# vocdoni/gnark-crypto-primitives

Hardware: AMD Instinct MI355X
Metric: proofs/sec, Arbo-160 Poseidon SMT-verifier circuit, Groth16/BN254 (higher is better)
Workload: dtype u32x8 Montgomery (254-bit integer)

## Files before the change

gnark_crypto_primitives_amd/csrc/solve.hip:

```cpp
#include <cstdlib>

#include "zkmi_internal.h"
#include "emul.h"
#include "ff29.h"
#include "ff29_asm.h"
#include "modinv30.h"

namespace zk {

__device__ __forceinline__ Fr fmul(const Fr& a, const Fr& b) {
  Fr r;
  pack_canonical<Fr29Params>(r.v,
                             mul_asm(unpack29<Fr29Params>(a.v), unpack29<Fr29Params>(b.v)));
  return r;
}
__device__ __forceinline__ Fr f_one() {
  Fr r;
#pragma unroll
  for (int i = 0; i < 8; i++) r.v[i] = Fr29Params::k261(i);
  return r;
}
__device__ Fr finv(const Fr& a) {
  Fr t, c;
  modinv30<ModInvFr>(t.v, a.v);
// ... 20 lines not shown
__device__ __forceinline__ uint32_t limb_at(const Fr& v, uint32_t pos, uint32_t wd) {
  if (pos >= 256) return 0;
  const uint32_t lo = v.v[pos >> 5], hi = (pos >> 5) < 7 ? v.v[(pos >> 5) + 1] : 0u;
  const uint64_t two = ((uint64_t)hi << 32) | lo;
  return (uint32_t)(two >> (pos & 31)) & ((1u << wd) - 1u);
}


template <int BANK, bool WAIT, bool NT>
__device__ __forceinline__ void st_acc(Fr* base, size_t row, size_t b, size_t Bp, const Fr& x) {
  uint4* p0 = reinterpret_cast<uint4*>(base) + row * 2 * Bp + b;
  uint4* p1 = p0 + Bp;
#define ZK_ST_ACC_ASM(A0, A1, A2, A3, A4, A5, A6, A7, LO, HI, NT_)                                 \
  asm volatile("v_accvgpr_write_b32 " A0 ", %2\n v_accvgpr_write_b32 " A1 ", %3\n"                 \
               "v_accvgpr_write_b32 " A2 ", %4\n v_accvgpr_write_b32 " A3 ", %5\n"                 \
               "v_accvgpr_write_b32 " A4 ", %6\n v_accvgpr_write_b32 " A5 ", %7\n"                 \
               "v_accvgpr_write_b32 " A6 ", %8\n v_accvgpr_write_b32 " A7 ", %9\n s_nop 1\n"       \
               "global_store_dwordx4 %0, " LO ", off" NT_ "\n"                                      \
               " global_store_dwordx4 %1, " HI ", off" NT_                                         \
               :: "v"(p0), "v"(p1), "v"(x.v[0]), "v"(x.v[1]), "v"(x.v[2]), "v"(x.v[3]),            \
                  "v"(x.v[4]), "v"(x.v[5]), "v"(x.v[6]), "v"(x.v[7])                               \
               : A0, A1, A2, A3, A4, A5, A6, A7, "memory")
#define ZK_ST_ACC(A0, A1, A2, A3, A4, A5, A6, A7, LO, HI)                                         \
  if (WAIT) asm volatile("s_waitcnt vmcnt(0)" ::: "memory");                                       \
  if constexpr (NT)                                                                                \
    ZK_ST_ACC_ASM(A0, A1, A2, A3, A4, A5, A6, A7, LO, HI, " nt");                                  \
  else                                                                                             \
    ZK_ST_ACC_ASM(A0, A1, A2, A3, A4, A5, A6, A7, LO, HI, "")
  if (BANK == 0) {
    ZK_ST_ACC("a0", "a1", "a2", "a3", "a4", "a5", "a6", "a7", "a[0:3]", "a[4:7]");
  } else if (BANK == 1) {
    ZK_ST_ACC("a8", "a9", "a10", "a11", "a12", "a13", "a14", "a15", "a[8:11]", "a[12:15]");
  } else if (BANK == 2) {
    ZK_ST_ACC("a16", "a17", "a18", "a19", "a20", "a21", "a22", "a23", "a[16:19]", "a[20:23]");
  } else {
    ZK_ST_ACC("a24", "a25", "a26", "a27", "a28", "a29", "a30", "a31", "a[24:27]", "a[28:31]");
  }
#undef ZK_ST_ACC
#undef ZK_ST_ACC_ASM
}

__device__ __forceinline__ Fr ld_sel(const Fr* slots, const Fr* consts, uint32_t i, bool is_const,
                                     size_t lane, size_t Bp) {
  const uint4* p0 = is_const ? reinterpret_cast<const uint4*>(consts + i)
                             : reinterpret_cast<const uint4*>(slots) + (size_t)i * 2 * Bp + lane;
  const uint4* p1 = p0 + (is_const ? (size_t)1 : Bp);
  const uint4 lo = *p0, hi = *p1;
  Fr r;
  r.v[0] = lo.x; r.v[1] = lo.y; r.v[2] = lo.z; r.v[3] = lo.w;
  r.v[4] = hi.x; r.v[5] = hi.y; r.v[6] = hi.z; r.v[7] = hi.w;
  return r;
}

template <int S, bool EMUL>
__global__ __launch_bounds__(64) void solve_vliw_kernel(const uint4* __restrict__ prog,
                                                        const Fr* __restrict__ consts, Fr* slots,
                                                        Fr* __restrict__ a, Fr* __restrict__ b,
                                                        Fr* __restrict__ c,
                                                        int32_t* __restrict__ status, size_t Bp,
                                                        uint32_t n_rows, uint32_t row_begin,
                                                        uint32_t row_end) {
  constexpr int PPW = 64 / S;
  const uint32_t sl = threadIdx.x / PPW;
  const size_t lane = (size_t)blockIdx.x * PPW + (threadIdx.x % PPW);
  int32_t st = 0;
#define LD(i) bi_ld(slots, (i), lane, Bp)
#define ST(i, v) bi_st(slots, (i), lane, Bp, (v))
#define STA(i, v) st_acc<0, true, false>(slots, (i), lane, Bp, (v))
#define LDSEL(i, isc) ld_sel(slots, consts, (i), (isc), lane, Bp)
  constexpr uint32_t CH = S > 32 ? 8 : S > 16 ? 16 : 32, RQ = 1 + S, CQ = CH * RQ, NX = (CQ + 63) / 64;
  __shared__ uint4 pq[CQ];
  const uint32_t total_q = n_rows * RQ;
  uint4 nx[NX];
  uint32_t cur = 0xffffffffu, pre = 0xffffffffu;
  for (uint32_t r = row_begin; r < row_end; r++) {
    const uint32_t ci = r / CH;
    if (ci != cur) {
      if (ci != pre) {
#pragma unroll
        for (uint32_t i = 0; i < NX; i++) {
          const uint32_t o = i * 64 + threadIdx.x, gq = ci * CQ + o;
          nx[i] = (o < CQ && gq < total_q) ? prog[gq] : make_uint4(0, 0, 0, 0);
        }
      }
#pragma unroll
      for (uint32_t i = 0; i < NX; i++) {
        const uint32_t o = i * 64 + threadIdx.x;
        if (o < CQ) pq[o] = nx[i];
      }
      cur = ci;
      pre = ci + 1;
#pragma unroll
      for (uint32_t i = 0; i < NX; i++) {
        const uint32_t o = i * 64 + threadIdx.x, gq = pre * CQ + o;
        nx[i] = (o < CQ && gq < total_q) ? prog[gq] : make_uint4(0, 0, 0, 0);
      }
      __syncthreads();
    }
    const uint32_t rr = r - ci * CH;
    const uint4 q = pq[(r - ci * CH) * RQ + 1 + sl];
    const uint32_t cls = __builtin_amdgcn_readfirstlane(vq_cls(q.x));
    const uint32_t op = vq_op(q.x), k = vq_k(q.x);
    const uint32_t d = q.y, x = q.z, y = q.w;
    switch (cls) {
      case CLS_M:
        if (op != OP_END) {
          const bool kc = op == OP_MULC || op == OP_FMAC, fma = op == OP_FMA || op == OP_FMAC;
          const Fr va = LD(x);
          const Fr vb = LDSEL(y, kc);
          const Fr vz = LD(fma ? k : x);
          Fr vc = fmul(va, vb);
          if (fma) vc = add(vc, vz);
          STA(d, vc);
          if (op == OP_MULABC) {
            st_acc<1, false, true>(a, k, lane, Bp, va);
            st_acc<2, false, true>(b, k, lane, Bp, vb);
            st_acc<3, false, true>(c, k, lane, Bp, vc);
          }
        }
        break;
      case CLS_X:
        if (op != OP_END) {
          const Fr va = LD(x), vb = LD(y);
          const Fr ab = fmul(va, vb);
          const Fr ab2 = add(ab, ab);
          STA(d, sub(add(va, vb), ab2));
          if (op == OP_XORABC) {
            st_acc<1, false, true>(a, k, lane, Bp, add(va, va));
            st_acc<2, false, true>(b, k, lane, Bp, vb);
            st_acc<3, false, true>(c, k, lane, Bp, ab2);
          }
        }
        break;
      case CLS_A:
        if (op != OP_END) {
          const bool kc = op == OP_SETC || op == OP_ADDC;
          const bool two = kc || op == OP_ADD || op == OP_SUB;
          const Fr va = LD(x);
          const Fr vb = LDSEL(two ? y : x, kc);
          Fr v;
          if (op == OP_SETC)
            v = vb;
          else if (op == OP_ADD || op == OP_ADDC)
            v = add(va, vb);
          else if (op == OP_SUB)
            v = sub(va, vb);
          else if (op == OP_NEG)
            v = neg(va);
          else
            v = va;
          STA(d, v);
        }
        break;
      case CLS_R:
        if (op != OP_END) {
          const Fr va = LD(d), vb = LD(x), vc = LD(y);
          st_acc<1, true, true>(a, k, lane, Bp, va);
          st_acc<2, false, true>(b, k, lane, Bp, vb);
          st_acc<3, false, true>(c, k, lane, Bp, vc);
          if (vq_assert(q.x) && fmul(va, vb) != vc) st = ZKMI_ERR_UNSATISFIED;
        }
        break;
      case CLS_I:
        if (op == OP_BXOR || op == OP_BAND) {
          const Fr pa = f_plain(LD(x)), pb = f_plain(LD(y));
          STA(d, f_small(op == OP_BXOR ? (pa.v[0] ^ pb.v[0]) : (pa.v[0] & pb.v[0])));
        } else if (op != OP_END) {
          const Fr va = LD(x), vy = LD(op == OP_DIV ? y : x);
          STA(d, op == OP_DIV ? fmul(va, finv(vy)) : finv(va));
        }
        break;
      case CLS_BITS: {
        const uint4 q0 = prog[(size_t)r * (1 + S) + 1];
        const uint32_t n = vbits_count(q0.w), wd = __builtin_amdgcn_readfirstlane(vbits_width(q0.w));
        const uint32_t per = (n + S - 1) / S;
        const uint32_t i0 = sl * per, i1 = i0 + per < n ? i0 + per : n;
        const Fr v = f_plain(LD(q0.z));
        const Fr one = f_one(), zero = Fr::zero();
        if (wd <= 1) {
          for (uint32_t i = i0; i < i1; i++) {
            const uint32_t bit = i < 256 ? (v.v[i >> 5] >> (i & 31)) & 1u : 0u;
            ST(q0.y + i, bit ? one : zero);
          }
        } else {
          for (uint32_t i = i0; i < i1; i++) ST(q0.y + i, f_small(limb_at(v, i * wd, wd)));
        }
        __builtin_amdgcn_s_waitcnt(0x0F70);
        break;
      }
      case CLS_BINV: {
        const uint4 hdr = prog[(size_t)r * (1 + S)];
        const uint32_t nrows = __builtin_amdgcn_readfirstlane(hdr.z);
        const uint4* pr = prog + (size_t)(r + 1) * (1 + S) + 1 + sl;
        Fr acc = f_one();
        for (uint32_t t = 0; t < nrows; t++) {
          const uint4 p = pr[(size_t)t * (1 + S)];
          if (vq_op(p.x) != OP_PAIR) continue;
          const Fr v = LD(p.z);
          ST(p.y, acc);
          if (!v.is_zero()) acc = fmul(acc, v);
        }
        Fr inv = finv(acc);
        for (uint32_t t = nrows; t-- > 0;) {
          const uint4 p = pr[(size_t)t * (1 + S)];
          if (vq_op(p.x) != OP_PAIR) continue;
          const Fr v = LD(p.z);
          if (v.is_zero()) {
            ST(p.y, Fr::zero());
          } else {
            const Fr res = fmul(inv, LD(p.y));
            inv = fmul(inv, v);
            ST(p.y, res);
// ... 38 lines not shown
          r += nrows;
          __builtin_amdgcn_s_waitcnt(0x0F70);
        } else if (hcls == CLS_LIMBS) {
          if (op == OP_BITS) {
            const uint32_t n = vbits_count(y), wd = vbits_width(y) ? vbits_width(y) : 1u;
            const Fr v = f_plain(LD(x));
            for (uint32_t i = 0; i < n; i++) ST(d + i, f_small(limb_at(v, i * wd, wd)));
          }
          __builtin_amdgcn_s_waitcnt(0x0F70);
        } else if constexpr (EMUL) {
          if (hcls == CLS_EMUL) {
            const uint4 q0 = prog[(size_t)r * (1 + S) + 1];
            const uint32_t nk = vemul_nout(aux) - 4, na = vemul_na(aux), c0 = vemul_const0(aux);
            if (sl == 0) {
              uint32_t A[12], B[12], T[24], Rm[9], P[8];
#pragma unroll
              for (int i = 0; i < 12; i++) A[i] = B[i] = 0;
              const uint4* pr = prog + (size_t)(r + 1) * (1 + S) + 1;
              for (uint32_t t = 0; t < nq; t++) {
                const uint4 p = pr[(size_t)(t / S) * (1 + S) + (t % S)];
                if (vq_op(p.x) != OP_HQ) continue;
                const Fr v = f_plain(LD(p.z));
                if (t < na)
                  emul_acc_at(A, v.v, t);
                else
                  emul_acc_at(B, v.v, t - na);
              }
#pragma unroll
              for (int i = 0; i < 4; i++) {
                const Fr v = f_plain(consts[c0 + i]);
                P[2 * i] = v.v[0];
                P[2 * i + 1] = v.v[1];
              }
              emul_mul(T, A, B);
              emul_divmod(T, Rm, P);
#pragma unroll
              for (int j = 0; j < 8; j++)
                if ((uint32_t)j < nk) ST(q0.y + j, f_small(T[2 * j], T[2 * j + 1]));
#pragma unroll
              for (int j = 0; j < 4; j++) ST(q0.y + nk + j, f_small(Rm[2 * j], Rm[2 * j + 1]));
            }
            r += nrows;
            __builtin_amdgcn_s_waitcnt(0x0F70);
          }
        }
        break;
      }
    }
    __builtin_amdgcn_fence(__ATOMIC_SEQ_CST, "wavefront");
  }
#undef LD
#undef ST
#undef STA
#undef LDSEL
  if (st) atomicMin(&status[lane], st);
}

__global__ void fill_one_row(Fr* row, size_t Bp) {
  size_t i = (size_t)blockIdx.x * blockDim.x + threadIdx.x;
  if (i < Bp) bi_st(row, 0, i, Bp, f_one());
}

__global__ __launch_bounds__(256) void scale_rows_kernel(Fr* base, size_t rows, size_t Bp, Fr k) {
  size_t i = (size_t)blockIdx.x * blockDim.x + threadIdx.x;
  const size_t stride = (size_t)gridDim.x * blockDim.x, total = rows * Bp;
  for (; i < total; i += stride) {
    const size_t row = i / Bp, l = i % Bp;
    bi_st(base, row, l, Bp, mul(bi_ld(base, row, l, Bp), k));
  }
}
__global__ __launch_bounds__(256) void scale_array_kernel(Fr* a, size_t n, Fr k) {
  size_t i = (size_t)blockIdx.x * blockDim.x + threadIdx.x;
  if (i < n) a[i] = mul(a[i], k);
}
static Fr k_to_f() {
  Fr k;
  for (int i = 0; i < 8; i++) k.v[i] = Fr29Params::k261(i);
  return k;
}
static Fr k_to_std() {
  Fr k = Fr::zero();
  k.v[7] = 1u << 27;
  return k;
}
static int scale_rows(zkmi_ctx* ctx, Fr* base, size_t rows, size_t Bp, const Fr& k) {
  if (rows == 0) return ZKMI_OK;
  size_t g = (rows * Bp + 255) / 256;
  if (g > 8192) g = 8192;
  hipLaunchKernelGGL(scale_rows_kernel, dim3((unsigned)g), dim3(256), 0, ctx->stream, base, rows,
                     Bp, k);
  ZK_HIP(hipGetLastError());
  return ZKMI_OK;
}
int rows_to_f_domain(zkmi_ctx* ctx, Fr* base, size_t rows, size_t Bp) {
  return scale_rows(ctx, base, rows, Bp, k_to_f());
}
int rows_to_std_domain(zkmi_ctx* ctx, Fr* base, size_t rows, size_t Bp) {
  return scale_rows(ctx, base, rows, Bp, k_to_std());
}
int array_to_f_domain(zkmi_ctx* ctx, Fr* a, size_t n) {
  if (n == 0) return ZKMI_OK;
  hipLaunchKernelGGL(scale_array_kernel, dim3((unsigned)((n + 255) / 256)), dim3(256), 0,
                     ctx->stream, a, n, k_to_f());
  ZK_HIP(hipGetLastError());
  return ZKMI_OK;
}

__global__ void zero_status(int32_t* st, size_t n) {
  size_t i = (size_t)blockIdx.x * blockDim.x + threadIdx.x;
  if (i < n) st[i] = 0;
}

int solve_init(zkmi_ctx* ctx, Fr* slots, int32_t* status, size_t Bp) {
  hipLaunchKernelGGL(fill_one_row, dim3((unsigned)(Bp / 64)), dim3(64), 0, ctx->stream, slots, Bp);
  hipLaunchKernelGGL(zero_status, dim3((unsigned)(Bp / 64)), dim3(64), 0, ctx->stream, status, Bp);
  ZK_HIP(hipGetLastError());
  return ZKMI_OK;
}

int solve_bi(zkmi_ctx* ctx, const zkmi_cs* cs, Fr* slots, Fr* a, Fr* b, Fr* c, int32_t* status,
             size_t Bp) {
  int rc = solve_init(ctx, slots, status, Bp);
  if (rc) return rc;
  return solve_rows(ctx, cs, slots, a, b, c, status, Bp, 0, cs->n_rows);
}

template <int S>
static void launch_solve(zkmi_ctx* ctx, const zkmi_cs* cs, Fr* slots, Fr* a, Fr* b, Fr* c,
                         int32_t* status, size_t Bp, uint32_t row_begin, uint32_t row_end) {
  hipLaunchKernelGGL((cs->has_emul ? solve_vliw_kernel<S, true> : solve_vliw_kernel<S, false>),
                     dim3((unsigned)(Bp * S / 64)), dim3(64), 0, ctx->stream,
                     (const uint4*)cs->program, cs->consts, slots, a, b, c, status, Bp, cs->n_rows,
                     row_begin, row_end);
}

int solve_rows(zkmi_ctx* ctx, const zkmi_cs* cs, Fr* slots, Fr* a, Fr* b, Fr* c, int32_t* status,
               size_t Bp, uint32_t row_begin, uint32_t row_end) {
  if (row_begin >= row_end) return ZKMI_OK;
  decltype(&launch_solve<1>) launch;
  switch (cs->lanes_per_proof) {
    case 1: launch = launch_solve<1>; break;
    case 2: launch = launch_solve<2>; break;
    case 4: launch = launch_solve<4>; break;
    case 8: launch = launch_solve<8>; break;
    case 16: launch = launch_solve<16>; break;
    case 32: launch = launch_solve<32>; break;
    case 64: launch = launch_solve<64>; break;
    default:
      ctx->err = "cs: lanes_per_proof must be a power of two, 1 .. 64";
      return ZKMI_ERR_ARG;
  }
  launch(ctx, cs, slots, a, b, c, status, Bp, row_begin, row_end);
  ZK_HIP(hipGetLastError());
  return ZKMI_OK;
}

}
```

gnark_crypto_primitives_amd/csrc/witness.hip:

```cpp
#include <algorithm>
#include <cstring>
#include <thread>

#include "zkmi_internal.h"
#include "ff29.h"
#if defined(__HIP_DEVICE_COMPILE__)
#include "ff29_asm.h"
#endif

using namespace zk;

namespace zk {

int pointer_kind(const void* p) {
  hipPointerAttribute_t attr;
  hipError_t e = hipPointerGetAttributes(&attr, p);
  if (e != hipSuccess) {
    (void)hipGetLastError();
    return PTR_PAGEABLE;
  }
  if (attr.type == hipMemoryTypeDevice || attr.type == hipMemoryTypeManaged) return PTR_DEVICE;
  if (attr.type == hipMemoryTypeHost) return PTR_PINNED;
  return PTR_PAGEABLE;
}
// ... 148 lines not shown
  Fr acc[3];
#pragma unroll
  for (int s = 0; s < 3; s++) {
    Fr sum = Fr::zero();
    const uint32_t lo = m.ptr[s][k], hi = m.ptr[s][k + 1];
    for (uint32_t j = lo; j < hi; j++) {
      const uint2 tm = m.terms[s][j];
      const Fr x = bi_ld(w, tm.x, p, Bp);
      const uint32_t kind = tm.y >> 30;
      if (kind == 1)
        sum = add(sum, x);
      else if (kind == 2)
        sum = sub(sum, x);
      else
        sum = add(sum, fmul_261(x, m.coeffs[tm.y & 0x3fffffffu]));
    }
    acc[s] = sum;
  }
  bi_st(a, k, p, Bp, acc[0]);
  bi_st(b, k, p, Bp, acc[1]);
  bi_st(c, k, p, Bp, acc[2]);
  if (mul(acc[0], acc[1]) != acc[2]) st[p] = ZKMI_ERR_UNSATISFIED;
  }
}

}

extern "C" {

void* zkmi_host_alloc(zkmi_ctx* ctx, size_t bytes) {
  if (!ctx || bytes == 0) return nullptr;
  if (hipSetDevice(ctx->device) != hipSuccess) return nullptr;
  void* p = nullptr;
  if (hipHostMalloc(&p, bytes, hipHostMallocDefault) != hipSuccess) {
    (void)hipGetLastError();
    ctx->err = "zkmi_host_alloc: hipHostMalloc(" + std::to_string(bytes) + " B) failed";
    return nullptr;
  }
  return p;
}

void zkmi_host_free(zkmi_ctx* ctx, void* p) {
  if (!p) return;
  if (ctx) hipSetDevice(ctx->device);
  hipHostFree(p);
}

int zkmi_set_copy_threads(zkmi_ctx* ctx, int threads) {
  if (!ctx || threads < 0 || threads > 64) return ZKMI_ERR_ARG;
  ctx->copy_threads = threads;
  return ZKMI_OK;
}

void zkmi_r1cs_free(zkmi_ctx* ctx, zkmi_r1cs* m) {
  if (!m) return;
  if (ctx) {
    hipSetDevice(ctx->device);
    hipStreamSynchronize(ctx->stream);
    sync_side_streams(ctx);
  }
  for (int s = 0; s < 3; s++) {
    if (m->ptr[s]) hipFree(m->ptr[s]);
    if (m->terms[s]) hipFree(m->terms[s]);
  }
  if (m->coeffs) hipFree(m->coeffs);
  delete m;
}

int zkmi_r1cs_load(zkmi_ctx* ctx, const zkmi_r1cs_desc* d, zkmi_r1cs** out) {
  ZK_HIP(hipSetDevice(ctx->device));
  if (!d || !out) return ZKMI_ERR_ARG;
  *out = nullptr;
  if (d->n_constraints == 0 || d->n_wires == 0 || d->n_coeffs == 0 || d->n_coeffs >= (1u << 30) ||
      !d->coeffs) {
    ctx->err = "r1cs: n_constraints, n_wires and n_coeffs (< 2^30) must be positive";
    return ZKMI_ERR_ARG;
  }
  std::vector<Fr> coeffs(d->n_coeffs);
  if (hipMemcpy(coeffs.data(), d->coeffs, (size_t)d->n_coeffs * 32, hipMemcpyDefault) != hipSuccess) {
    ctx->err = "r1cs: cannot read the coefficient table";
    return ZKMI_ERR_HIP;
  }
  const Fr one = Fr::one(), minus_one = neg(Fr::one());
  std::vector<uint8_t> kind(d->n_coeffs);
  for (uint32_t i = 0; i < d->n_coeffs; i++) {
    const Fr& x = coeffs[i];
    bool lt = false;
    for (int j = 7; j >= 0; j--) {
      if (x.v[j] != FrParams::p(j)) {
        lt = x.v[j] < FrParams::p(j);
        break;
      }
    }
    if (!lt) {
      ctx->err = "r1cs: coefficient " + std::to_string(i) + " is not reduced mod r";
      return ZKMI_ERR_ARG;
    }
    kind[i] = x == one ? 1 : x == minus_one ? 2 : 0;
  }
  auto* m = new zkmi_r1cs();
  m->n_wires = d->n_wires;
  m->n_constraints = d->n_constraints;
  m->n_coeffs = d->n_coeffs;
  const uint32_t* ptrs[3] = {d->l_ptr, d->r_ptr, d->o_ptr};
  const zkmi_term* terms[3] = {d->l_terms, d->r_terms, d->o_terms};
  static const char* names[3] = {"L", "R", "O"};
// ... 143 lines not shown
```

gnark_crypto_primitives_amd/csrc/zkmi_internal.h:

```cpp
#pragma once
#include <hip/hip_runtime.h>
#include <stdint.h>
#include <string>
#include <utility>
#include <vector>

#include "../../include/zkmi.h"
#include "ec.h"
#include "vprog.h"

namespace zk {


struct DevBuf {
  void* p = nullptr;
  size_t bytes = 0;
};

struct NttPlan {
  int log_n = 0;
  Fr* tw_fwd = nullptr;
  Fr* tw_inv = nullptr;
  Fr* coset_fwd = nullptr;
  Fr* coset_inv = nullptr;
// ... 9 lines not shown

}

struct zkmi_ctx {
  int device = 0;
  hipStream_t stream = nullptr;
  std::string err;
  std::vector<zk::NttPlan> plans;
  hipEvent_t ev[8] = {};
  double timings[8] = {};
  zk::DevBuf ntt_tmp;
  zk::DevBuf ntt_top;
  zk::DevBuf build_tmp;
  zk::DevBuf msm_digits, msm_sint;
  zk::DevBuf msm_rowvar;
  zk::DevBuf msm_part[2];
  zk::DevBuf side_part2;
  zk::DevBuf side_part3;
  hipStream_t stream2 = nullptr, stream3 = nullptr, stream4 = nullptr;
  struct ProveSet {
    bool pending = false;
    bool heavy_enqueued = false;
    zk::DevBuf slots, a, b, c, misc, sums, commit;
    hipEvent_t evq[5] = {};
    hipEvent_t eva[2] = {};
    hipEvent_t tail_ev = nullptr;
    hipEvent_t msm_ev[8][2] = {};
    int msm_ev_group[8] = {};
    int msm_ev_used = 0;
    size_t batch = 0, Bp = 0;
    const zkmi_pk* pk = nullptr;
    const zkmi_cs* cs = nullptr;
    size_t n_constraints = 0;
    bool f_domain = true;
    void *rs = nullptr, *st = nullptr;
    hipEvent_t ev0 = nullptr, ev1 = nullptr;
    void *commit_pts = nullptr, *commit_ch = nullptr, *commit_pok = nullptr, *commit_acc = nullptr;
    std::vector<zk::Fr> commit_host;
  } sets[2];
  int next_submit = 0, next_collect = 0;
  int msm_ev_set = -1;
  hipEvent_t part_ev[2] = {}, acc_ev[2] = {}, dig_ev[2] = {};
  bool part_ev_valid[2] = {false, false};
  unsigned part_next = 0;
  struct StageRing {
    void* pinned[3] = {};
    void* dev[3] = {};
    hipEvent_t done[3] = {};
    bool busy[3] = {false, false, false};
    size_t bytes = 0;
    unsigned next = 0;
  } ring;
  int copy_threads = 0;
};

struct WinPlan {
  int W = 0;
  uint32_t per_base = 0;
  uint8_t bits[64] = {};
  uint32_t off[64] = {};
  uint8_t shared = 0;
  uint8_t comb = 0;
  uint8_t comb_signed = 0;
};

struct zkmi_msm_bases {
  int group = 1;
  size_t n = 0;
  WinPlan plan;
  void* table = nullptr;
  size_t table_bytes = 0;
  uint8_t* inf = nullptr;
  size_t n_groups = 0;
  int entries_may_be_inf = 0;
  uint32_t chunk_factor = 0;
  int image = 0;
  zk::G1Affine stotal1 = {};
  zk::G2Affine stotal2 = {};
  int side = 0;
};

struct zkmi_commit_key {
  uint32_t n_private = 0, n_hashed = 0, wire = 0;
  std::vector<uint32_t> hashed;
  std::vector<uint32_t> priv;
  uint32_t* private_dev = nullptr;
  zkmi_msm_bases* basis = nullptr;
  zkmi_msm_bases* sigma = nullptr;
};

struct zkmi_pk {
  uint32_t log_n = 0, n_wires = 0, n_a = 0, n_b = 0, n_k = 0, n_z = 0, max_batch = 1024;
  uint32_t *a_wire = nullptr, *b_wire = nullptr, *k_wire = nullptr;
  zkmi_msm_bases *A = nullptr, *B1 = nullptr, *K = nullptr, *Z = nullptr, *B2 = nullptr;
  zkmi_msm_bases *D1 = nullptr, *D2 = nullptr;
  uint32_t* idx3 = nullptr;
  zk::G1Affine alpha, beta1, delta1;
  zk::G2Affine beta2, delta2;
  std::vector<zkmi_commit_key> commits;
  bool folded = false;
  uint32_t fold_n_constraints = 0;
};

struct zkmi_cs {
  uint32_t n_wires = 0, n_public = 0, n_secret = 0, n_constraints = 0, n_slots = 0, n_rows = 0,
           n_consts = 0, lanes_per_proof = 1;
// ... 193 lines not shown
```

gnark_crypto_primitives_amd/lib.py:

```python
from __future__ import annotations

import ctypes as C
import os

import numpy as np

_HERE = os.path.dirname(os.path.abspath(__file__))
LIB_PATH = os.environ.get("ZKMI_LIB", os.path.join(_HERE, "libzkmi.so"))

ZKMI_OK = 0
ZKMI_ERR_UNSATISFIED = -5


class ZkmiError(RuntimeError):
    pass


class PkDesc(C.Structure):
    _fields_ = [("log_n", C.c_uint32), ("n_wires", C.c_uint32), ("n_a", C.c_uint32),
                ("n_b", C.c_uint32), ("n_k", C.c_uint32), ("n_z", C.c_uint32),
                ("a_wire", C.c_void_p), ("b_wire", C.c_void_p), ("k_wire", C.c_void_p),
                ("g1_a", C.c_void_p), ("g1_b", C.c_void_p), ("g1_k", C.c_void_p),
                ("g1_z", C.c_void_p), ("g2_b", C.c_void_p), ("g1_alpha", C.c_void_p),
                ("g1_beta", C.c_void_p), ("g1_delta", C.c_void_p), ("g2_beta", C.c_void_p),
# ... 53 lines not shown
                ("n_hints", C.c_uint32), ("instr", C.c_void_p), ("hint_kind", C.c_void_p),
                ("hint_in_ptr", C.c_void_p), ("hint_in_wire", C.c_void_p),
                ("hint_in_coef", C.c_void_p), ("hint_out_ptr", C.c_void_p), ("hint_out", C.c_void_p),
                ("lanes_per_proof", C.c_uint32), ("hint_set", C.c_uint32)]


class PlonkCommitDesc(C.Structure):
    _fields_ = [("n_rows", C.c_uint32), ("row", C.c_uint32), ("rows", C.c_void_p),
                ("slots", C.c_void_p), ("lag_g1", C.c_void_p), ("lag_k", C.c_uint32)]


PLONK_MAX_COMMITMENTS = 8
HINTS_BASIC, HINTS_STD, HINTS_EMULATED = 0, 1, 3


_P, _SZ, _I = C.c_void_p, C.c_size_t, C.c_int
SYMBOLS = [
    ("zkmi_init", _I, [_I, C.POINTER(_P)]),
    ("zkmi_destroy", None, [_P]),
    ("zkmi_last_error", C.c_char_p, [_P]),
    ("zkmi_sync", _I, [_P]),
    ("zkmi_stream", _P, [_P]),
    ("zkmi_field_mul", _I, [_P, _I, _P, _P, _P, _SZ]),
    ("zkmi_ff29_op", _I, [_P, _I, _I, _P, _P, _SZ]),
    ("zkmi_field_mul_bench", _I, [_P, _I, _SZ, _I, C.POINTER(C.c_double)]),
    ("zkmi_ntt_batch", _I, [_P, _P, _I, _SZ, _I, _I]),
    ("zkmi_h_batch", _I, [_P, _P, _P, _P, _P, _I, _SZ]),
    ("zkmi_ab_coset_batch", _I, [_P, _P, _P, _P, _I, _SZ]),
    ("zkmi_quotient_bases", _I, [_P, _P, _SZ, _I, _P, _P]),
    ("zkmi_msm_bases_load", _I, [_P, _I, _P, _SZ, _I, C.POINTER(_P)]),
    ("zkmi_msm_bases_free", None, [_P, _P]),
    ("zkmi_msm_batch", _I, [_P, _P, _P, _SZ, _P]),
    ("zkmi_msm_bases_load_image", _I, [_P, _I, _P, _SZ, _I, _I, C.POINTER(_P)]),
    ("zkmi_msm_batch_rows", _I, [_P, _P, _P, _SZ, _P, _SZ, _I, _I, _P]),
    ("zkmi_comb_min_groups_per_chunk", C.c_uint32, []),
    ("zkmi_fixed_base_mul", _I, [_P, _I, _P, _P, _SZ, _P]),
    ("zkmi_pk_load", _I, [_P, C.POINTER(PkDesc), C.POINTER(_P)]),
    ("zkmi_pk_free", None, [_P, _P]),
    ("zkmi_pk_load_planned", _I, [_P, C.POINTER(PkDesc), C.POINTER(C.c_uint32), C.POINTER(_P)]),
    ("zkmi_pk_info", _I, [_P, C.POINTER(C.c_uint64)]),
    ("zkmi_pk_msm_plan", _I, [_P, C.POINTER(C.c_uint32)]),
    ("zkmi_pk_folded", _I, [_P]),
    ("zkmi_cs_load", _I, [_P, C.POINTER(CsDesc), C.POINTER(_P)]),
    ("zkmi_cs_free", None, [_P, _P]),
    ("zkmi_solve_batch", _I, [_P, _P, _P, _SZ, _P, _P, _P]),
    ("zkmi_prove_batch", _I, [_P, _P, _P, _P, _SZ, _P, _P, _P]),
    ("zkmi_prove_submit", _I, [_P, _P, _P, _P, _SZ, _P]),
    ("zkmi_prove_collect", _I, [_P, _P, _P]),
    ("zkmi_prove_collect_ex", _I, [_P, _P, _P, _P]),
    ("zkmi_prove_witness_batch", _I, [_P, _P, _P, _P, _P, _P, _SZ, _SZ, _P, _P]),
    ("zkmi_host_alloc", _P, [_P, _SZ]),
    ("zkmi_host_free", None, [_P, _P]),
    ("zkmi_set_copy_threads", _I, [_P, _I]),
    ("zkmi_r1cs_load", _I, [_P, C.POINTER(R1csDesc), C.POINTER(_P)]),
    ("zkmi_r1cs_free", None, [_P, _P]),
    ("zkmi_prove_witness_submit", _I, [_P, _P, _P, _P, _P, _P, _P, _SZ, _SZ, _P]),
    ("zkmi_r1cs_solver_load", _I, [_P, _P, C.POINTER(R1csSolverDesc), C.POINTER(_P)]),
    ("zkmi_r1cs_solver_free", None, [_P, _P]),
    ("zkmi_r1cs_solver_info", _I, [_P, C.POINTER(C.c_uint64)]),
    ("zkmi_r1cs_solve_batch", _I, [_P, _P, _P, _SZ, _P, _P, _P]),
    ("zkmi_prove_r1cs_submit", _I, [_P, _P, _P, _P, _SZ, _P]),
    ("zkmi_last_timings", _I, [_P, C.POINTER(C.c_double)]),
    ("zkmi_plonk_pk_load", _I, [_P, _P, C.POINTER(_P)]),
    ("zkmi_plonk_pk_free", None, [_P, _P]),
    ("zkmi_plonk_round1", _I, [_P, _P, _P, _P, _SZ, _P, _P, _P]),
    ("zkmi_plonk_round2", _I, [_P, _P, _P, _P]),
    ("zkmi_plonk_round3", _I, [_P, _P, _P, _P]),
    ("zkmi_plonk_round4", _I, [_P, _P, _P, _P]),
    ("zkmi_plonk_round5", _I, [_P, _P, _P, _P]),
    ("zkmi_plonk_prove", _I, [_P, _P, _P, _P, _SZ, _P, _P, _P, _P]),
    ("zkmi_plonk_pk_load_trace", _I, [_P, C.POINTER(PlonkTraceDesc), C.POINTER(_P)]),
    ("zkmi_scs_load", _I, [_P, C.POINTER(ScsDesc), C.POINTER(_P)]),
    ("zkmi_scs_free", None, [_P, _P]),
    ("zkmi_plonk_round1_witness", _I, [_P, _P, _P, _P, _P, _P, _P, _SZ, _SZ, _P, _P, _P]),
    ("zkmi_plonk_prove_witness", _I, [_P, _P, _P, _P, _P, _P, _P, _SZ, _SZ, _P, _P, _P, _P]),
    ("zkmi_plonk_pk_set_commitments", _I, [_P, _P, C.POINTER(PlonkCommitDesc), C.c_uint32]),
    ("zkmi_plonk_commit_hint", _I, [_P, _P, C.c_uint32, _P, _P, _SZ, _P, _P]),
    ("zkmi_plonk_prove_ex", _I, [_P, _P, _P, _P, _SZ, _P, _P, _P, _P, _P, _P]),
    ("zkmi_plonk_prove_witness_ex", _I, [_P, _P, _P, _P, _P, _P, _P, _SZ, _SZ, _P, _P, _P, _P, _P,
                                         _P]),
    ("zkmi_scs_solver_load", _I, [_P, _P, C.POINTER(ScsSolverDesc), C.POINTER(_P)]),
    ("zkmi_scs_solver_free", None, [_P, _P]),
    ("zkmi_scs_solver_info", _I, [_P, C.POINTER(C.c_uint64)]),
    ("zkmi_scs_solve_batch", _I, [_P, _P, _P, _SZ, _P, _P]),
    ("zkmi_plonk_round1_scs", _I, [_P, _P, _P, _P, _SZ, _P, _P, _P]),
    ("zkmi_plonk_prove_scs", _I, [_P, _P, _P, _P, _SZ, _P, _P, _P, _P]),
]

_lib = None


def load():
    global _lib
    if _lib is not None:
        return _lib
    if not os.path.exists(LIB_PATH):
        raise ZkmiError(f"{LIB_PATH} not found: build it with `python -c 'import __graft_entry__ as "
                        "g; g.build()'` (hipcc --offload-arch=gfx950). There is no CPU fallback.")
    lib = C.CDLL(LIB_PATH)
    for name, res, args in SYMBOLS:
        fn = getattr(lib, name)
        fn.restype = res
        fn.argtypes = args
    _lib = lib
    return lib

# ... 237 lines not shown
                    "zkmi_plonk_pk_load_trace")
        return h

    def scs_load(self, desc: "ScsDesc"):
        h = C.c_void_p()
        self._check(self.lib.zkmi_scs_load(self.h, C.byref(desc), C.byref(h)), "zkmi_scs_load")
        return h

    def scs_free(self, h):
        self.lib.zkmi_scs_free(self.h, h)

    def scs_solver_load(self, scs_h, desc: "ScsSolverDesc"):
        h = C.c_void_p()
        self._check(self.lib.zkmi_scs_solver_load(self.h, scs_h, C.byref(desc), C.byref(h)),
                    "zkmi_scs_solver_load")
        return h

    def scs_solver_free(self, h):
        self.lib.zkmi_scs_solver_free(self.h, h)

    def scs_solver_info(self, h):
        arr = (C.c_uint64 * 8)()
        self._check(self.lib.zkmi_scs_solver_info(h, arr), "zkmi_scs_solver_info")
        return dict(zip(("n_instr", "lanes_per_proof", "n_records", "n_steps", "n_inversions",
                         "n_wires", "n_gates", "n_inputs"), [int(x) for x in arr]))

    def scs_solve_batch(self, solver_h, inputs, batch, wires_out=None, status_out=None):
        if status_out is None:
            status_out = np.zeros(batch, dtype=np.int32)
        self._check(self.lib.zkmi_scs_solve_batch(self.h, solver_h, _ptr(inputs), batch,
                                                  _ptr(wires_out), _ptr(status_out)),
                    "zkmi_scs_solve_batch")
        return status_out

    def host_alloc(self, shape, dtype=np.uint64):
        nbytes = int(np.prod(shape)) * np.dtype(dtype).itemsize
        p = self.lib.zkmi_host_alloc(self.h, nbytes)
        if not p:
            raise ZkmiError(f"zkmi_host_alloc({nbytes}) failed")
        buf = (C.c_uint8 * nbytes).from_address(p)
        arr = np.frombuffer(buf, dtype=dtype).reshape(shape)
        self._pinned = getattr(self, "_pinned", {})
        self._pinned[arr.ctypes.data] = p
        return arr

    def host_free(self, arr):
        p = getattr(self, "_pinned", {}).pop(arr.ctypes.data, None)
        if p:
            self.lib.zkmi_host_free(self.h, p)

    def set_copy_threads(self, n):
        self._check(self.lib.zkmi_set_copy_threads(self.h, n), "zkmi_set_copy_threads")

    def last_timings(self):
        arr = (C.c_double * 8)()
        self.lib.zkmi_last_timings(self.h, arr)
        return list(arr)
```

include/zkmi.h:

```cpp
#ifndef ZKMI_H
#define ZKMI_H
#include <stddef.h>
#include <stdint.h>

#ifdef __cplusplus
extern "C" {
#endif

typedef struct zkmi_ctx zkmi_ctx;
typedef struct zkmi_pk zkmi_pk;
typedef struct zkmi_cs zkmi_cs;
typedef struct zkmi_r1cs_desc zkmi_r1cs_desc;

enum zkmi_status {
  ZKMI_OK = 0,
  ZKMI_ERR_ARG = -1,
  ZKMI_ERR_HIP = -2,
  ZKMI_ERR_NO_DEVICE = -3,
  ZKMI_ERR_OOM = -4,
  ZKMI_ERR_UNSATISFIED = -5
};

int zkmi_init(int device, zkmi_ctx** out);
void zkmi_destroy(zkmi_ctx* ctx);
// ... 54 lines not shown
  const void* g2_b;
  const void* g1_alpha;
  const void* g1_beta;
  const void* g1_delta;
  const void* g2_beta;
  const void* g2_delta;
  uint32_t window_bits_g1;
  uint32_t window_bits_g2;
  const uint8_t* infinity_a;
  const uint8_t* infinity_b;
  uint32_t n_public;
  uint32_t max_batch;
  uint64_t table_budget_bytes;
  uint32_t n_slots_hint;
  uint32_t msm_chunk_factor;
  uint32_t sparse_witness;
  uint32_t n_commitments;
  const zkmi_commitment_desc* commitments;
  const zkmi_r1cs_desc* fold_r1cs;
} zkmi_pk_desc;
int zkmi_pk_load(zkmi_ctx* ctx, const zkmi_pk_desc* desc, zkmi_pk** out);
int zkmi_pk_load_planned(zkmi_ctx* ctx, const zkmi_pk_desc* desc, const uint32_t* msm_window_bits,
                         zkmi_pk** out);
void zkmi_pk_free(zkmi_ctx* ctx, zkmi_pk* pk);
int zkmi_pk_info(const zkmi_pk* pk, uint64_t* info );
int zkmi_pk_msm_plan(const zkmi_pk* pk, uint32_t* plan );
int zkmi_pk_folded(const zkmi_pk* pk);

typedef struct {
  uint32_t n_wires, n_public, n_secret, n_constraints;
  uint32_t n_slots, n_rows, n_consts;
  uint32_t lanes_per_proof;
  const uint32_t* program;
  const void* consts;
} zkmi_cs_desc;
int zkmi_cs_load(zkmi_ctx* ctx, const zkmi_cs_desc* desc, zkmi_cs** out);
void zkmi_cs_free(zkmi_ctx* ctx, zkmi_cs* cs);

int zkmi_solve_batch(zkmi_ctx* ctx, const zkmi_cs* cs, const void* inputs, size_t batch,
                     void* wires_out, void* abc_out, int32_t* status_out);

int zkmi_prove_batch(zkmi_ctx* ctx, const zkmi_pk* pk, const zkmi_cs* cs, const void* inputs,
                     size_t batch, const void* rs, void* proofs_out, int32_t* status_out);

int zkmi_prove_submit(zkmi_ctx* ctx, const zkmi_pk* pk, const zkmi_cs* cs, const void* inputs,
                      size_t batch, const void* rs);
int zkmi_prove_collect(zkmi_ctx* ctx, void* proofs_out, int32_t* status_out);
int zkmi_prove_collect_ex(zkmi_ctx* ctx, void* proofs_out, int32_t* status_out,
                          void* commitments_out);

void* zkmi_host_alloc(zkmi_ctx* ctx, size_t bytes);
void zkmi_host_free(zkmi_ctx* ctx, void* p);
int zkmi_set_copy_threads(zkmi_ctx* ctx, int threads);

typedef struct {
  uint32_t coeff;
  uint32_t wire;
} zkmi_term;
struct zkmi_r1cs_desc {
  uint32_t n_wires, n_constraints, n_coeffs;
  const void* coeffs;
  const uint32_t* l_ptr;
  const zkmi_term* l_terms;
  const uint32_t* r_ptr;
  const zkmi_term* r_terms;
  const uint32_t* o_ptr;
  const zkmi_term* o_terms;
};
typedef struct zkmi_r1cs zkmi_r1cs;
int zkmi_r1cs_load(zkmi_ctx* ctx, const zkmi_r1cs_desc* desc, zkmi_r1cs** out);
void zkmi_r1cs_free(zkmi_ctx* ctx, zkmi_r1cs* r1cs);

int zkmi_prove_witness_submit(zkmi_ctx* ctx, const zkmi_pk* pk, const zkmi_r1cs* r1cs,
                              const void* wires, const void* a, const void* b, const void* c,
                              size_t n_constraints, size_t batch, const void* rs);
int zkmi_prove_witness_batch(zkmi_ctx* ctx, const zkmi_pk* pk, const void* wires, const void* a,
                             const void* b, const void* c, size_t n_constraints, size_t batch,
                             const void* rs, void* proofs_out);

enum zkmi_hint_kind {
  ZKMI_HINT_INVZERO = 1,
  ZKMI_HINT_NBITS = 2,
  ZKMI_HINT_LIMBS = 3,
  ZKMI_HINT_COUNT = 4,
  ZKMI_HINT_COMMIT = 5,
  ZKMI_HINT_BYTEOP = 6,
  ZKMI_HINT_EMULMUL = 7
};
enum zkmi_hint_set {
  ZKMI_HINTS_BASIC = 0,
  ZKMI_HINTS_STD = 1,
  ZKMI_HINTS_EMULATED = 3
};
typedef struct {
  uint32_t n_public;
  uint32_t n_secret;
  uint32_t n_instr, n_hints;
  const uint32_t* instr;
  const uint32_t* hint_kind;
  const uint32_t* hint_in_ptr;
  const uint32_t* hint_lc_ptr;
  const zkmi_term* hint_terms;
  const uint32_t* hint_out_ptr;
  const uint32_t* hint_out;
  uint32_t lanes_per_proof;
  uint32_t hint_set;
// ... 134 lines not shown
```

Baseline: 9234.

## Pack several independent solver wavefronts per workgroup in the VLIW solve kernel

The witness solver used to launch one 64-thread workgroup per wavefront. The default path now packs up to 4 (or 8) independent wavefronts into one workgroup, each with its own shared-memory program chunk. Each wave synchronises with a wavefront fence and wave barrier instead of __syncthreads. With 8 waves per block the accumulator-register store path is replaced by plain or non-temporal stores. This aims to cut per-workgroup scheduling overhead and raise occupancy, at the cost of larger LDS use per block and possible register-pressure changes.

```diff
diff --git a/gnark_crypto_primitives_amd/csrc/solve.hip b/gnark_crypto_primitives_amd/csrc/solve.hip
--- a/gnark_crypto_primitives_amd/csrc/solve.hip
+++ b/gnark_crypto_primitives_amd/csrc/solve.hip
@@ -96,24 +96,38 @@
   return r;
 }
 
-template <int S, bool EMUL>
-__global__ __launch_bounds__(64) void solve_vliw_kernel(const uint4* __restrict__ prog,
-                                                        const Fr* __restrict__ consts, Fr* slots,
-                                                        Fr* __restrict__ a, Fr* __restrict__ b,
-                                                        Fr* __restrict__ c,
-                                                        int32_t* __restrict__ status, size_t Bp,
-                                                        uint32_t n_rows, uint32_t row_begin,
-                                                        uint32_t row_end) {
+template <int S>
+struct SolveChunk {
+  static constexpr uint32_t CH = S > 32 ? 8 : S > 16 ? 16 : 32, RQ = 1 + S, CQ = CH * RQ,
+                            NX = (CQ + 63) / 64;
+};
+
+template <int S, bool EMUL, int MAXW>
+__device__ __forceinline__ void solve_vliw_wave(
+    uint4* const pq, const uint32_t tl, const size_t wave, const uint4* __restrict__ prog,
+    const Fr* __restrict__ consts, Fr* slots, Fr* __restrict__ a, Fr* __restrict__ b,
+    Fr* __restrict__ c, int32_t* __restrict__ status, size_t Bp, uint32_t n_rows, uint32_t row_begin,
+    uint32_t row_end) {
   constexpr int PPW = 64 / S;
-  const uint32_t sl = threadIdx.x / PPW;
-  const size_t lane = (size_t)blockIdx.x * PPW + (threadIdx.x % PPW);
+  constexpr bool PACKED = MAXW > 1, ACC = MAXW <= 4;
+  const uint32_t sl = tl / PPW;
+  const size_t lane = wave * PPW + (tl % PPW);
   int32_t st = 0;
 #define LD(i) bi_ld(slots, (i), lane, Bp)
 #define ST(i, v) bi_st(slots, (i), lane, Bp, (v))
-#define STA(i, v) st_acc<0, true, false>(slots, (i), lane, Bp, (v))
+#define STR(BANK, WAIT, NT, base, row, v)                          \
+  do {                                                               \
+    if constexpr (ACC)                                               \
+      st_acc<BANK, WAIT, NT>((base), (row), lane, Bp, (v));          \
+    else if constexpr (NT)                                           \
+      bi_st_nt((base), (row), lane, Bp, (v));                        \
+    else                                                             \
+      bi_st((base), (row), lane, Bp, (v));                           \
+  } while (0)
+#define STA(i, v) STR(0, true, false, slots, (i), (v))
 #define LDSEL(i, isc) ld_sel(slots, consts, (i), (isc), lane, Bp)
-  constexpr uint32_t CH = S > 32 ? 8 : S > 16 ? 16 : 32, RQ = 1 + S, CQ = CH * RQ, NX = (CQ + 63) / 64;
-  __shared__ uint4 pq[CQ];
+  constexpr uint32_t CH = SolveChunk<S>::CH, RQ = SolveChunk<S>::RQ, CQ = SolveChunk<S>::CQ,
+                     NX = SolveChunk<S>::NX;
   const uint32_t total_q = n_rows * RQ;
   uint4 nx[NX];
   uint32_t cur = 0xffffffffu, pre = 0xffffffffu;
@@ -123,23 +137,28 @@
       if (ci != pre) {
 #pragma unroll
         for (uint32_t i = 0; i < NX; i++) {
-          const uint32_t o = i * 64 + threadIdx.x, gq = ci * CQ + o;
+          const uint32_t o = i * 64 + tl, gq = ci * CQ + o;
           nx[i] = (o < CQ && gq < total_q) ? prog[gq] : make_uint4(0, 0, 0, 0);
         }
       }
 #pragma unroll
       for (uint32_t i = 0; i < NX; i++) {
-        const uint32_t o = i * 64 + threadIdx.x;
+        const uint32_t o = i * 64 + tl;
         if (o < CQ) pq[o] = nx[i];
       }
       cur = ci;
       pre = ci + 1;
 #pragma unroll
       for (uint32_t i = 0; i < NX; i++) {
-        const uint32_t o = i * 64 + threadIdx.x, gq = pre * CQ + o;
+        const uint32_t o = i * 64 + tl, gq = pre * CQ + o;
         nx[i] = (o < CQ && gq < total_q) ? prog[gq] : make_uint4(0, 0, 0, 0);
       }
-      __syncthreads();
+      if constexpr (!PACKED) {
+        __syncthreads();
+      } else {
+        __builtin_amdgcn_fence(__ATOMIC_SEQ_CST, "wavefront");
+        __builtin_amdgcn_wave_barrier();
+      }
     }
     const uint32_t rr = r - ci * CH;
     const uint4 q = pq[(r - ci * CH) * RQ + 1 + sl];
@@ -157,9 +176,9 @@
           if (fma) vc = add(vc, vz);
           STA(d, vc);
           if (op == OP_MULABC) {
-            st_acc<1, false, true>(a, k, lane, Bp, va);
-            st_acc<2, false, true>(b, k, lane, Bp, vb);
-            st_acc<3, false, true>(c, k, lane, Bp, vc);
+            STR(1, false, true, a, k, va);
+            STR(2, false, true, b, k, vb);
+            STR(3, false, true, c, k, vc);
           }
         }
         break;
@@ -170,9 +189,9 @@
           const Fr ab2 = add(ab, ab);
           STA(d, sub(add(va, vb), ab2));
           if (op == OP_XORABC) {
-            st_acc<1, false, true>(a, k, lane, Bp, add(va, va));
-            st_acc<2, false, true>(b, k, lane, Bp, vb);
-            st_acc<3, false, true>(c, k, lane, Bp, ab2);
+            STR(1, false, true, a, k, add(va, va));
+            STR(2, false, true, b, k, vb);
+            STR(3, false, true, c, k, ab2);
           }
         }
         break;
@@ -199,9 +218,9 @@
       case CLS_R:
         if (op != OP_END) {
           const Fr va = LD(d), vb = LD(x), vc = LD(y);
-          st_acc<1, true, true>(a, k, lane, Bp, va);
-          st_acc<2, false, true>(b, k, lane, Bp, vb);
-          st_acc<3, false, true>(c, k, lane, Bp, vc);
+          STR(1, true, true, a, k, va);
+          STR(2, false, true, b, k, vb);
+          STR(3, false, true, c, k, vc);
           if (vq_assert(q.x) && fmul(va, vb) != vc) st = ZKMI_ERR_UNSATISFIED;
         }
         break;
@@ -346,8 +365,35 @@
 #undef LD
 #undef ST
 #undef STA
+#undef STR
 #undef LDSEL
   if (st) atomicMin(&status[lane], st);
+}
+
+template <int S, bool EMUL>
+__global__ __launch_bounds__(64) void solve_vliw_kernel(const uint4* __restrict__ prog,
+                                                        const Fr* __restrict__ consts, Fr* slots,
+                                                        Fr* __restrict__ a, Fr* __restrict__ b,
+                                                        Fr* __restrict__ c,
+                                                        int32_t* __restrict__ status, size_t Bp,
+                                                        uint32_t n_rows, uint32_t row_begin,
+                                                        uint32_t row_end) {
+  __shared__ uint4 pq[SolveChunk<S>::CQ];
+  solve_vliw_wave<S, EMUL, 1>(pq, threadIdx.x, blockIdx.x, prog, consts, slots, a, b, c, status,
+                                  Bp, n_rows, row_begin, row_end);
+}
+
+template <int S, bool EMUL, int MAXW>
+__global__ __launch_bounds__(64 * MAXW) void solve_vliw_packed_kernel(
+    const uint4* __restrict__ prog, const Fr* __restrict__ consts, Fr* slots, Fr* __restrict__ a,
+    Fr* __restrict__ b, Fr* __restrict__ c, int32_t* __restrict__ status, size_t Bp, uint32_t n_rows,
+    uint32_t row_begin, uint32_t row_end, uint32_t waves) {
+  __shared__ uint4 pq_all[MAXW][SolveChunk<S>::CQ];
+  const uint32_t wv = threadIdx.x / 64;
+  const uint32_t wave = blockIdx.x * (blockDim.x / 64) + wv;
+  if (wave >= waves) return;
+  solve_vliw_wave<S, EMUL, MAXW>(pq_all[wv], threadIdx.x % 64, wave, prog, consts, slots, a, b, c,
+                                 status, Bp, n_rows, row_begin, row_end);
 }
 
 __global__ void fill_one_row(Fr* row, size_t Bp) {
@@ -419,13 +465,25 @@
   return solve_rows(ctx, cs, slots, a, b, c, status, Bp, 0, cs->n_rows);
 }
 
+static constexpr unsigned SOLVE_WAVES_DEFAULT = 4;
 template <int S>
 static void launch_solve(zkmi_ctx* ctx, const zkmi_cs* cs, Fr* slots, Fr* a, Fr* b, Fr* c,
                          int32_t* status, size_t Bp, uint32_t row_begin, uint32_t row_end) {
-  hipLaunchKernelGGL((cs->has_emul ? solve_vliw_kernel<S, true> : solve_vliw_kernel<S, false>),
-                     dim3((unsigned)(Bp * S / 64)), dim3(64), 0, ctx->stream,
+  const unsigned wpb = ctx->solve_waves ? ctx->solve_waves : SOLVE_WAVES_DEFAULT;
+  const unsigned waves = (unsigned)(Bp * S / 64);
+  if (wpb == 1) {
+    hipLaunchKernelGGL((cs->has_emul ? solve_vliw_kernel<S, true> : solve_vliw_kernel<S, false>),
+                       dim3(waves), dim3(64), 0, ctx->stream, (const uint4*)cs->program, cs->consts,
+                       slots, a, b, c, status, Bp, cs->n_rows, row_begin, row_end);
+    return;
+  }
+  auto kernel = wpb > 4 ? (cs->has_emul ? solve_vliw_packed_kernel<S, true, 8>
+                                        : solve_vliw_packed_kernel<S, false, 8>)
+                        : (cs->has_emul ? solve_vliw_packed_kernel<S, true, 4>
+                                        : solve_vliw_packed_kernel<S, false, 4>);
+  hipLaunchKernelGGL(kernel, dim3((waves + wpb - 1) / wpb), dim3(64 * wpb), 0, ctx->stream,
                      (const uint4*)cs->program, cs->consts, slots, a, b, c, status, Bp, cs->n_rows,
-                     row_begin, row_end);
+                     row_begin, row_end, waves);
 }
 
 int solve_rows(zkmi_ctx* ctx, const zkmi_cs* cs, Fr* slots, Fr* a, Fr* b, Fr* c, int32_t* status,
diff --git a/gnark_crypto_primitives_amd/csrc/witness.hip b/gnark_crypto_primitives_amd/csrc/witness.hip
--- a/gnark_crypto_primitives_amd/csrc/witness.hip
+++ b/gnark_crypto_primitives_amd/csrc/witness.hip
@@ -224,6 +224,13 @@
   return ZKMI_OK;
 }
 
+int zkmi_set_solve_waves_per_block(zkmi_ctx* ctx, int waves) {
+  if (!ctx || (waves != 0 && waves != 1 && waves != 2 && waves != 4 && waves != 8))
+    return ZKMI_ERR_ARG;
+  ctx->solve_waves = waves;
+  return ZKMI_OK;
+}
+
 void zkmi_r1cs_free(zkmi_ctx* ctx, zkmi_r1cs* m) {
   if (!m) return;
   if (ctx) {
diff --git a/gnark_crypto_primitives_amd/csrc/zkmi_internal.h b/gnark_crypto_primitives_amd/csrc/zkmi_internal.h
--- a/gnark_crypto_primitives_amd/csrc/zkmi_internal.h
+++ b/gnark_crypto_primitives_amd/csrc/zkmi_internal.h
@@ -85,6 +85,7 @@
     unsigned next = 0;
   } ring;
   int copy_threads = 0;
+  int solve_waves = 0;
 };
 
 struct WinPlan {
diff --git a/gnark_crypto_primitives_amd/lib.py b/gnark_crypto_primitives_amd/lib.py
--- a/gnark_crypto_primitives_amd/lib.py
+++ b/gnark_crypto_primitives_amd/lib.py
@@ -129,6 +129,7 @@
     ("zkmi_host_alloc", _P, [_P, _SZ]),
     ("zkmi_host_free", None, [_P, _P]),
     ("zkmi_set_copy_threads", _I, [_P, _I]),
+    ("zkmi_set_solve_waves_per_block", _I, [_P, _I]),
     ("zkmi_r1cs_load", _I, [_P, C.POINTER(R1csDesc), C.POINTER(_P)]),
     ("zkmi_r1cs_free", None, [_P, _P]),
     ("zkmi_prove_witness_submit", _I, [_P, _P, _P, _P, _P, _P, _P, _SZ, _SZ, _P]),
@@ -472,6 +473,12 @@
     def set_copy_threads(self, n):
         self._check(self.lib.zkmi_set_copy_threads(self.h, n), "zkmi_set_copy_threads")
 
+    def set_solve_waves_per_block(self, w):
+        rc = self.lib.zkmi_set_solve_waves_per_block(self.h, w)
+        if rc != 0:
+            raise ZkmiError(f"zkmi_set_solve_waves_per_block({w}) refused ({rc}): "
+                            "0 (default), 1, 2, 4 or 8")
+
     def last_timings(self):
         arr = (C.c_double * 8)()
         self.lib.zkmi_last_timings(self.h, arr)
diff --git a/include/zkmi.h b/include/zkmi.h
--- a/include/zkmi.h
+++ b/include/zkmi.h
@@ -130,6 +130,7 @@
 void* zkmi_host_alloc(zkmi_ctx* ctx, size_t bytes);
 void zkmi_host_free(zkmi_ctx* ctx, void* p);
 int zkmi_set_copy_threads(zkmi_ctx* ctx, int threads);
+int zkmi_set_solve_waves_per_block(zkmi_ctx* ctx, int waves);
 
 typedef struct {
   uint32_t coeff;
```

Result: faster. 9789 (median of 6 runs) (+6.0%).
